# Aleph-Alpha/magma

Measured on NVIDIA H100. Metric: image-caption samples/sec (fwd+bwd), higher is better.
Workload: dtype bf16

## Files before the change

### magma_b200/csrc/attention.cu

```cuda
#include <stdlib.h>

#include "gemm_common.cuh"

namespace mb200 {

static constexpr int kAttThreads = 256;
static constexpr int kTile = 128 * 64 * 2;

struct AttnParams {
  int S, H, hd, rot;
  float scale;
  bf16* P;
  long long ldP;
  bf16* O;
  long long ldo;
  bf16* dqkv;
  long long ld_dqkv;
  const float2* rope_tab;
  const bf16* dPe;
  long long ld_dpe;
};

__device__ __forceinline__ void fence_async_smem() { asm volatile("fence.proxy.async.shared::cta;" ::: "memory"); }
__device__ __forceinline__ void wg_sync(int wg) { asm volatile("bar.sync %0, 128;" ::"r"(wg + 1) : "memory"); }

__device__ __forceinline__ uint32_t operand_off(int r, int c) {
  return (uint32_t)((c >> 6) * kTile + r * 128 + ((((c & 63) >> 3) ^ (r & 7)) << 4) + (c & 7) * 2);
}
__device__ __forceinline__ void st_pair(uint32_t saddr, float a, float b) {
  asm volatile("st.shared.b32 [%0], %1;" ::"r"(saddr), "r"(f32x2_to_bf16(a, b)) : "memory");
}
__device__ __forceinline__ float2 ld_pair(uint32_t saddr) {
  uint32_t u;
  asm volatile("ld.shared.b32 %0, [%1];" : "=r"(u) : "r"(saddr));
  return bf16x2_to_f32(u);
}
__device__ __forceinline__ float quad_max(float v) {
  v = fmaxf(v, __shfl_xor_sync(0xffffffffu, v, 1));
  return fmaxf(v, __shfl_xor_sync(0xffffffffu, v, 2));
}
__device__ __forceinline__ float quad_sum(float v) {
  v += __shfl_xor_sync(0xffffffffu, v, 1);
  return v + __shfl_xor_sync(0xffffffffu, v, 2);
}

template <int N, bool A_MN, bool B_MN>
__device__ __forceinline__ void wg_mma(float (&d)[N / 2], int wg, uint32_t a_base, uint32_t b_base, int nkb,
                                       uint32_t acc0 = 0u) {
  a_base += A_MN ? (uint32_t)(wg * kTile) : (uint32_t)(wg * 64 * 128);
  wgmma_fence();
  for (int kb = 0; kb < nkb; ++kb) {
#pragma unroll
    for (int k = 0; k < 4; ++k) {
      const uint32_t ao = A_MN ? (uint32_t)((kb * 4 + k) * 2048) : (uint32_t)(kb * kTile + k * 32);
      const uint32_t bo = B_MN ? (uint32_t)((kb * 4 + k) * 2048) : (uint32_t)(kb * kTile + k * 32);
      const uint64_t da = make_smem_desc(a_base + ao, A_MN ? (uint32_t)kTile : 0u, 1024);
      const uint64_t db = make_smem_desc(b_base + bo, B_MN ? (uint32_t)kTile : 0u, 1024);
      wgmma_bf16<N, A_MN ? 1 : 0, B_MN ? 1 : 0>(d, da, db, ((kb | k) != 0 ? 1u : 0u) | acc0);
    }
  }
  wgmma_commit();
  wgmma_wait<0>();
}

struct Frag {
  int wg, r0, c0, quad0;
  __device__ __forceinline__ Frag() {
    const int t = threadIdx.x;
    wg = t >> 7;
    r0 = wg * 64 + ((t & 127) >> 5) * 16 + ((t & 31) >> 2);
    c0 = 2 * (t & 3);
    quad0 = (t & 3) == 0;
  }
};

template <int HD>
__device__ __forceinline__ void store_rows(const Frag& f, const float (&d)[HD / 2], bf16* dst, long long ld, int nrows,
                                           const float2* tab, int rot) {
#pragma unroll
  for (int h = 0; h < 2; ++h) {
    const int r = f.r0 + 8 * h;
    if (r >= nrows) continue;
    bf16* row = dst + (long long)r * ld;
#pragma unroll
    for (int j = 0; j < HD / 8; ++j) {
      const int c = 8 * j + f.c0;
      float a0 = d[4 * j + 2 * h], a1 = d[4 * j + 2 * h + 1];
      if (tab != nullptr && c < rot) {
        const float2 cs = __ldg(tab + (long long)r * (rot >> 1) + (c >> 1));
        const float b0 = a0 * cs.x + a1 * cs.y;
        a1 = a1 * cs.x - a0 * cs.y;
        a0 = b0;
      }
      *reinterpret_cast<uint32_t*>(row + c) = f32x2_to_bf16(a0, a1);
    }
  }
}

template <int HD>
__global__ void __launch_bounds__(kAttThreads, 1)
attn_fwd_tile_kernel(const __grid_constant__ CUtensorMap tmQ, const __grid_constant__ CUtensorMap tmK,
                     const __grid_constant__ CUtensorMap tmV, const AttnParams p) {
  extern __shared__ uint8_t smem_raw[];
  uint8_t* smem = reinterpret_cast<uint8_t*>((reinterpret_cast<uintptr_t>(smem_raw) + 1023) & ~uintptr_t(1023));
  constexpr int nhb = HD / 64;
  uint8_t* sQ = smem;
  uint8_t* sK = sQ + nhb * kTile;
  uint8_t* sV = sK + nhb * kTile;
  uint8_t* sP = sV + nhb * kTile;
  uint64_t* bars = reinterpret_cast<uint64_t*>(sP + 2 * kTile);
  uint64_t* bar_qk = bars + 0;
  uint64_t* bar_v = bars + 1;

  const int t = threadIdx.x;
  const int h = blockIdx.x % p.H, b = blockIdx.x / p.H;
  const Frag f;

  pdl_trigger();
  if (t == 0) {
    tma_prefetch_desc(&tmQ);
    tma_prefetch_desc(&tmK);
    tma_prefetch_desc(&tmV);
    for (int i = 0; i < 2; ++i) mbar_init(&bars[i], 1);
    mbar_fence_init();
  }
  __syncthreads();
  pdl_wait();

  if (t == 0) {
    mbar_expect_tx(bar_qk, 2 * nhb * kTile);
    for (int kb = 0; kb < nhb; ++kb) {
      tma_load_4d(sQ + kb * kTile, &tmQ, bar_qk, kb * 64, 0, h, b);
      tma_load_4d(sK + kb * kTile, &tmK, bar_qk, kb * 64, 0, h, b);
    }
    mbar_expect_tx(bar_v, nhb * kTile);
    for (int kb = 0; kb < nhb; ++kb) tma_load_4d(sV + kb * kTile, &tmV, bar_v, kb * 64, 0, h, b);
  }
  mbar_wait(bar_qk, 0);
  float s[64];
  wg_mma<128, false, false>(s, f.wg, smem_u32(sQ), smem_u32(sK), nhb);
  const uint32_t sP_s = smem_u32(sP);
#pragma unroll
  for (int hh = 0; hh < 2; ++hh) {
    const int q = f.r0 + 8 * hh;
    const int lim = min(p.S, q + 1);
    float m = -INFINITY;
#pragma unroll
    for (int j = 0; j < 16; ++j)
#pragma unroll
      for (int e = 0; e < 2; ++e) {
        float& v = s[4 * j + 2 * hh + e];
        v *= p.scale;
        if (8 * j + f.c0 + e < lim) m = fmaxf(m, v);
      }
    m = quad_max(m);
    float sum = 0.f;
#pragma unroll
    for (int j = 0; j < 16; ++j)
#pragma unroll
      for (int e = 0; e < 2; ++e) {
        float& v = s[4 * j + 2 * hh + e];
        v = 8 * j + f.c0 + e < lim ? __expf(v - m) : 0.f;
        sum += v;
      }
    sum = quad_sum(sum);
    const float inv = q < p.S ? 1.f / sum : 0.f;
    bf16* prow = p.P + (((long long)b * p.H + h) * p.S + q) * p.ldP;
#pragma unroll
    for (int j = 0; j < 16; ++j) {
      const int c = 8 * j + f.c0;
      const float a0 = s[4 * j + 2 * hh] * inv, a1 = s[4 * j + 2 * hh + 1] * inv;
      st_pair(sP_s + operand_off(q, c), a0, a1);
      if (q < p.S && c < p.ldP) *reinterpret_cast<uint32_t*>(prow + c) = f32x2_to_bf16(a0, a1);
    }
  }
  fence_async_smem();
  wg_sync(f.wg);
  mbar_wait(bar_v, 0);
  float o[HD / 2];
  wg_mma<HD, false, true>(o, f.wg, sP_s, smem_u32(sV), 2);
  store_rows<HD>(f, o, p.O + (long long)b * p.S * p.ldo + (long long)h * HD, p.ldo, p.S, nullptr, 0);
}

template <int HD, bool EXT_DP>
__global__ void __launch_bounds__(kAttThreads, 1)
attn_bwd_tile_kernel(const __grid_constant__ CUtensorMap tmQ, const __grid_constant__ CUtensorMap tmK,
                     const __grid_constant__ CUtensorMap tmV, const __grid_constant__ CUtensorMap tmdO,
                     const __grid_constant__ CUtensorMap tmP, const AttnParams p) {
  extern __shared__ uint8_t smem_raw[];
  uint8_t* smem = reinterpret_cast<uint8_t*>((reinterpret_cast<uintptr_t>(smem_raw) + 1023) & ~uintptr_t(1023));
  constexpr int nhb = HD / 64;
  uint8_t* R1 = smem;
  uint8_t* R2 = R1 + nhb * kTile;
  uint8_t* R3 = R2 + nhb * kTile;
  uint8_t* R4 = R3 + 2 * kTile;
  uint64_t* bars = reinterpret_cast<uint64_t*>(R4 + 2 * kTile);
  uint64_t* bar_a = bars + 0;
  uint64_t* bar_p = bars + 1;
  uint64_t* bar_k = bars + 2;
  uint64_t* bar_q = bars + 3;

  const int t = threadIdx.x;
  const int h = blockIdx.x % p.H, b = blockIdx.x / p.H;
  const Frag f;

  pdl_trigger();
  if (t == 0) {
    tma_prefetch_desc(&tmQ);
    tma_prefetch_desc(&tmK);
    tma_prefetch_desc(&tmV);
    tma_prefetch_desc(&tmdO);
    tma_prefetch_desc(&tmP);
    for (int i = 0; i < 4; ++i) mbar_init(&bars[i], 1);
    mbar_fence_init();
  }
  __syncthreads();
  pdl_wait();

  if (t == 0) {
    mbar_expect_tx(bar_a, 2 * nhb * kTile);
    for (int kb = 0; kb < nhb; ++kb) {
      tma_load_4d(R1 + kb * kTile, &tmdO, bar_a, kb * 64, 0, h, b);
      tma_load_4d(R2 + kb * kTile, &tmV, bar_a, kb * 64, 0, h, b);
    }
    mbar_expect_tx(bar_p, 2 * kTile);
    for (int kb = 0; kb < 2; ++kb) tma_load_4d(R3 + kb * kTile, &tmP, bar_p, kb * 64, 0, h, b);
  }
  const uint32_t R3_s = smem_u32(R3), R4_s = smem_u32(R4);
  {
    uint32_t ext[EXT_DP ? 32 : 1];
    if (EXT_DP) {
#pragma unroll
      for (int hh = 0; hh < 2; ++hh) {
        const int q = f.r0 + 8 * hh;
        const bf16* erow = p.dPe + (((long long)b * p.H + h) * p.S + q) * p.ld_dpe;
#pragma unroll
        for (int j = 0; j < 16; ++j) {
          const int c = 8 * j + f.c0;
          uint32_t v = 0u;
          if (q < p.S && c < p.S) {
            v = __ldg(reinterpret_cast<const unsigned int*>(erow + c));
            if (c + 1 >= p.S) v &= 0xffffu;
          }
          ext[16 * hh + j] = v;
        }
      }
    }
    mbar_wait(bar_a, 0);
    float dp[64];
    wg_mma<128, false, false>(dp, f.wg, smem_u32(R1), smem_u32(R2), nhb);
    if (EXT_DP) {
#pragma unroll
      for (int hh = 0; hh < 2; ++hh)
#pragma unroll
        for (int j = 0; j < 16; ++j) {
          const float2 e = bf16x2_to_f32(ext[16 * hh + j]);
          dp[4 * j + 2 * hh] += e.x;
          dp[4 * j + 2 * hh + 1] += e.y;
        }
    }
    mbar_wait(bar_p, 0);
#pragma unroll
    for (int hh = 0; hh < 2; ++hh) {
      const int q = f.r0 + 8 * hh;
      float acc = 0.f;
#pragma unroll
      for (int j = 0; j < 16; ++j) {
        const float2 pr = ld_pair(R3_s + operand_off(q, 8 * j + f.c0));
        acc += dp[4 * j + 2 * hh] * pr.x + dp[4 * j + 2 * hh + 1] * pr.y;
      }
      acc = quad_sum(acc);
#pragma unroll
      for (int j = 0; j < 16; ++j) {
        const uint32_t off = operand_off(q, 8 * j + f.c0);
        const float2 pr = ld_pair(R3_s + off);
        st_pair(R4_s + off, pr.x * (dp[4 * j + 2 * hh] - acc) * p.scale, pr.y * (dp[4 * j + 2 * hh + 1] - acc) * p.scale);
      }
    }
  }
  const long long HDall = (long long)p.H * HD;
  bf16* gbase = p.dqkv + (long long)b * p.S * p.ld_dqkv + (long long)h * HD;
  {
    float dv[HD / 2];
    wg_mma<HD, true, true>(dv, f.wg, R3_s, smem_u32(R1), 2);
    store_rows<HD>(f, dv, gbase + 2 * HDall, p.ld_dqkv, p.S, nullptr, 0);
  }
  fence_async_smem();
  __syncthreads();
  if (t == 0) {
    mbar_expect_tx(bar_k, nhb * kTile);
    for (int kb = 0; kb < nhb; ++kb) tma_load_4d(R2 + kb * kTile, &tmK, bar_k, kb * 64, 0, h, b);
    mbar_expect_tx(bar_q, nhb * kTile);
    for (int kb = 0; kb < nhb; ++kb) tma_load_4d(R1 + kb * kTile, &tmQ, bar_q, kb * 64, 0, h, b);
  }
  {
    mbar_wait(bar_k, 0);
    float dq[HD / 2];
    wg_mma<HD, false, true>(dq, f.wg, R4_s, smem_u32(R2), 2);
    store_rows<HD>(f, dq, gbase, p.ld_dqkv, p.S, p.rope_tab, p.rot);
  }
  {
    mbar_wait(bar_q, 0);
    float dk[HD / 2];
    wg_mma<HD, true, true>(dk, f.wg, R4_s, smem_u32(R1), 2);
    store_rows<HD>(f, dk, gbase + HDall, p.ld_dqkv, p.S, p.rope_tab, p.rot);
  }
}

struct FlashParams {
  int Sq, Sk, H, hd, causal, kv_off;
  float scale;
  bf16* O;
  long long ldo;
  bf16* P;
  long long ldP;
  float2* stats;
};

template <int HD, int NBUF>
__global__ void __launch_bounds__(kAttThreads, 1)
attn_fwd_flash_kernel(const __grid_constant__ CUtensorMap tmQ, const __grid_constant__ CUtensorMap tmK,
                      const __grid_constant__ CUtensorMap tmV, const FlashParams p) {
  extern __shared__ uint8_t smem_raw[];
  uint8_t* smem = reinterpret_cast<uint8_t*>((reinterpret_cast<uintptr_t>(smem_raw) + 1023) & ~uintptr_t(1023));
  constexpr int nhb = HD / 64;
  uint8_t* sQ = smem;
  uint8_t* sK = sQ + nhb * kTile;
  uint8_t* sV = sK + NBUF * nhb * kTile;
  uint8_t* sP = sV + NBUF * nhb * kTile;
  uint64_t* bars = reinterpret_cast<uint64_t*>(sP + 2 * kTile);
  uint64_t* bar_q = bars + 0;
  uint64_t* bar_k = bars + 1;
  uint64_t* bar_v = bars + 3;

  const int t = threadIdx.x;
  const int q0 = blockIdx.x * 128, h = blockIdx.y, b = blockIdx.z;
  const Frag f;

  pdl_trigger();
  if (t == 0) {
    tma_prefetch_desc(&tmQ);
    tma_prefetch_desc(&tmK);
    tma_prefetch_desc(&tmV);
    for (int i = 0; i < 5; ++i) mbar_init(&bars[i], 1);
    mbar_fence_init();
  }
  __syncthreads();
  pdl_wait();

  int n_kv = (p.Sk + 127) >> 7;
  if (p.causal) {
    const int last_key = min(p.Sk - 1, q0 + 127 + p.kv_off);
    n_kv = last_key < 0 ? 0 : min(n_kv, (last_key >> 7) + 1);
  }
  int row_lim[2];
  bool row_ok[2];
#pragma unroll
  for (int hh = 0; hh < 2; ++hh) {
    const int qi = q0 + f.r0 + 8 * hh;
    row_lim[hh] = !p.causal ? p.Sk : min(p.Sk, qi + p.kv_off + 1);
    row_ok[hh] = qi < p.Sq;
  }

  uint32_t ph_k[2] = {0, 0}, ph_v[2] = {0, 0};
  auto load_k = [&](int j, int buf) {
    mbar_expect_tx(&bar_k[buf], nhb * kTile);
    for (int kb = 0; kb < nhb; ++kb) tma_load_4d(sK + (buf * nhb + kb) * kTile, &tmK, &bar_k[buf], kb * 64, j * 128, h, b);
  };
  auto load_v = [&](int j, int buf) {
    mbar_expect_tx(&bar_v[buf], nhb * kTile);
    for (int kb = 0; kb < nhb; ++kb) tma_load_4d(sV + (buf * nhb + kb) * kTile, &tmV, &bar_v[buf], kb * 64, j * 128, h, b);
  };

  float m[2] = {-INFINITY, -INFINITY}, l[2] = {0.f, 0.f};
  if (t == 0 && n_kv > 0) {
    mbar_expect_tx(bar_q, nhb * kTile);
    for (int kb = 0; kb < nhb; ++kb) tma_load_4d(sQ + kb * kTile, &tmQ, bar_q, kb * 64, q0, h, b);
    load_k(0, 0);
  }
  if (n_kv > 0) mbar_wait(bar_q, 0);
  float s[64];
  for (int j = 0; j < n_kv; ++j) {
    const int buf = NBUF == 2 ? (j & 1) : 0;
    if (t == 0) {
      if (NBUF == 2 && j + 1 < n_kv) load_k(j + 1, (j + 1) & 1);
      if (NBUF == 1 && j + 1 < n_kv)
        for (int kb = 0; kb < nhb; ++kb) tma_prefetch_4d(&tmK, kb * 64, (j + 1) * 128, h, b);
    }
    mbar_wait(&bar_k[buf], ph_k[buf]);
    ph_k[buf] ^= 1;
    wg_mma<128, false, false>(s, f.wg, smem_u32(sQ), smem_u32(sK + buf * nhb * kTile), nhb);
    __syncthreads();
    if (NBUF == 1 && t == 0 && j + 1 < n_kv) load_k(j + 1, 0);
    const int kbase = j * 128;
#pragma unroll
    for (int hh = 0; hh < 2; ++hh) {
      float cm = -INFINITY;
#pragma unroll
      for (int jj = 0; jj < 16; ++jj)
#pragma unroll
        for (int e = 0; e < 2; ++e)
          if (kbase + 8 * jj + f.c0 + e < row_lim[hh]) cm = fmaxf(cm, s[4 * jj + 2 * hh + e] * p.scale);
      cm = quad_max(cm);
      if (cm > m[hh]) {
        l[hh] *= __expf(m[hh] - cm);
        m[hh] = cm;
      }
      if (m[hh] != -INFINITY) {
        float ls = 0.f;
#pragma unroll
        for (int jj = 0; jj < 16; ++jj)
#pragma unroll
          for (int e = 0; e < 2; ++e)
            if (kbase + 8 * jj + f.c0 + e < row_lim[hh]) ls += __expf(s[4 * jj + 2 * hh + e] * p.scale - m[hh]);
        l[hh] += quad_sum(ls);
      }
    }
  }
  float inv[2];
#pragma unroll
  for (int hh = 0; hh < 2; ++hh) {
    inv[hh] = (row_ok[hh] && l[hh] > 0.f) ? 1.f / l[hh] : 0.f;
    if (m[hh] == -INFINITY) m[hh] = 0.f;
    if (p.stats != nullptr && row_ok[hh] && f.quad0)
      p.stats[((long long)b * p.H + h) * p.Sq + q0 + f.r0 + 8 * hh] = make_float2(m[hh], inv[hh]);
  }

  const uint32_t sP_s = smem_u32(sP);
  if (t == 0 && n_kv > 0) {
    load_k(0, 0);
    load_v(0, 0);
  }
  float o[HD / 2];
#pragma unroll
  for (int i = 0; i < HD / 2; ++i) o[i] = 0.f;
  for (int j = 0; j < n_kv; ++j) {
    const int buf = NBUF == 2 ? (j & 1) : 0;
    if (t == 0) {
      if (NBUF == 2 && j + 1 < n_kv) {
        load_k(j + 1, (j + 1) & 1);
        load_v(j + 1, (j + 1) & 1);
      }
      if (NBUF == 1 && j + 1 < n_kv)
        for (int kb = 0; kb < nhb; ++kb) {
          tma_prefetch_4d(&tmK, kb * 64, (j + 1) * 128, h, b);
          tma_prefetch_4d(&tmV, kb * 64, (j + 1) * 128, h, b);
        }
    }
    mbar_wait(&bar_k[buf], ph_k[buf]);
    ph_k[buf] ^= 1;
    wg_mma<128, false, false>(s, f.wg, smem_u32(sQ), smem_u32(sK + buf * nhb * kTile), nhb);
    __syncthreads();
    if (NBUF == 1 && t == 0 && j + 1 < n_kv) load_k(j + 1, 0);
    const int kbase = j * 128;
#pragma unroll
    for (int hh = 0; hh < 2; ++hh) {
      const int r = f.r0 + 8 * hh;
      bf16* prow = p.P ? p.P + (((long long)b * p.H + h) * p.Sq + q0 + r) * p.ldP : nullptr;
#pragma unroll
      for (int jj = 0; jj < 16; ++jj) {
        const int c = 8 * jj + f.c0;
        float a[2];
#pragma unroll
        for (int e = 0; e < 2; ++e)
          a[e] = kbase + c + e < row_lim[hh] ? __expf(s[4 * jj + 2 * hh + e] * p.scale - m[hh]) * inv[hh] : 0.f;
        st_pair(sP_s + operand_off(r, c), a[0], a[1]);
        if (prow != nullptr && row_ok[hh] && kbase + c < p.ldP)
          *reinterpret_cast<uint32_t*>(prow + kbase + c) = f32x2_to_bf16(a[0], a[1]);
      }
    }
    fence_async_smem();
    wg_sync(f.wg);
    mbar_wait(&bar_v[buf], ph_v[buf]);
    ph_v[buf] ^= 1;
    wg_mma<HD, false, true>(o, f.wg, sP_s, smem_u32(sV + buf * nhb * kTile), 2, 1u);
    __syncthreads();
    if (NBUF == 1 && t == 0 && j + 1 < n_kv) load_v(j + 1, 0);
  }
  store_rows<HD>(f, o, p.O + ((long long)b * p.Sq + q0) * p.ldo + (long long)h * HD, p.ldo, p.Sq - q0, nullptr, 0);
  if (p.P != nullptr && t < 128 && q0 + t < p.Sq) {
    bf16* prow = p.P + (((long long)b * p.H + h) * p.Sq + q0 + t) * p.ldP;
    for (int col = n_kv * 128; col < p.ldP; col += 8) *reinterpret_cast<uint4*>(prow + col) = make_uint4(0, 0, 0, 0);
  }
}

static int tile_map(CUtensorMap* m, const void* ptr, long long ld, long long bs0, long long bs1, int rows, int cols,
                    int H, int B) {
  mb200_operand op;
  op.ptr = ptr;
  op.ld = ld;
  op.bs0 = bs0;
  op.bs1 = bs1;
  op.mn_major = 0;
  op.static_data = 0;
  return make_operand_map(m, op, rows, cols, H, B, 128);
}

static constexpr int smem_max = 232448;

bool attn_tile_supported(int S, int hd) { return S >= 1 && S <= 128 && hd >= 64 && hd <= 256 && hd % 64 == 0; }

int attn_fwd_tile(const bf16* qkv, long long ld_qkv, bf16* P, long long ldP, bf16* O, long long ldo, int B, int S, int H,
                  int hd, cudaStream_t st) {
  MB_REQUIRE(attn_tile_supported(S, hd) && ldP % 8 == 0, MB200_E_SHAPE, "attn_fwd_tile: unsupported S=%d hd=%d", S, hd);
  CUtensorMap tq, tk, tv;
  const long long d = (long long)H * hd;
  int rc;
  if ((rc = tile_map(&tq, qkv, ld_qkv, hd, (long long)S * ld_qkv, S, hd, H, B))) return rc;
  if ((rc = tile_map(&tk, qkv + d, ld_qkv, hd, (long long)S * ld_qkv, S, hd, H, B))) return rc;
  if ((rc = tile_map(&tv, qkv + 2 * d, ld_qkv, hd, (long long)S * ld_qkv, S, hd, H, B))) return rc;
  AttnParams p;
  memset(&p, 0, sizeof(p));
  p.S = S;
  p.H = H;
  p.hd = hd;
  p.scale = 1.0f / sqrtf((float)hd);
  p.P = P;
  p.ldP = ldP;
  p.O = O;
  p.ldo = ldo;
  const int smem = (3 * (hd / 64) + 2) * kTile + 1024 + 128;
#define MB_FWD(HD)                                                                                                   \
  {                                                                                                                  \
    static bool set = false;                                                                                         \
    if (!set) {                                                                                                      \
      MB_CUDA(cudaFuncSetAttribute(attn_fwd_tile_kernel<HD>, cudaFuncAttributeMaxDynamicSharedMemorySize, smem_max)); \
      set = true;                                                                                                    \
    }                                                                                                                \
    MB_CUDA(launch_pdl(attn_fwd_tile_kernel<HD>, dim3(B * H), dim3(kAttThreads), (size_t)smem, st, tq, tk, tv, p));  \
  }
  switch (hd) {
    case 64: MB_FWD(64) break;
    case 128: MB_FWD(128) break;
    case 192: MB_FWD(192) break;
    default: MB_FWD(256) break;
  }
#undef MB_FWD
  count_launch();
  return 0;
}

int attn_bwd_tile(const bf16* qkv, long long ld_qkv, const bf16* dO, long long ld_do, const bf16* P, long long ldP,
                  const bf16* dPe, long long ld_dpe, bf16* dqkv, long long ld_dqkv, const float* rope_tab, int rot, int B,
                  int S, int H, int hd, cudaStream_t st) {
  MB_REQUIRE(attn_tile_supported(S, hd) && ldP % 8 == 0, MB200_E_SHAPE, "attn_bwd_tile: unsupported S=%d hd=%d", S, hd);
  MB_REQUIRE(dPe == nullptr || (ld_dpe >= S && ld_dpe % 8 == 0 && (reinterpret_cast<uintptr_t>(dPe) & 3) == 0),
             MB200_E_ALIGN, "attn_bwd_tile_dp: ld_dpe=%lld must be >= S and %%8, dP_ext 4-byte aligned", ld_dpe);
  CUtensorMap tq, tk, tv, tdo, tp;
  const long long d = (long long)H * hd;
  int rc;
  if ((rc = tile_map(&tq, qkv, ld_qkv, hd, (long long)S * ld_qkv, S, hd, H, B))) return rc;
  if ((rc = tile_map(&tk, qkv + d, ld_qkv, hd, (long long)S * ld_qkv, S, hd, H, B))) return rc;
  if ((rc = tile_map(&tv, qkv + 2 * d, ld_qkv, hd, (long long)S * ld_qkv, S, hd, H, B))) return rc;
  if ((rc = tile_map(&tdo, dO, ld_do, hd, (long long)S * ld_do, S, hd, H, B))) return rc;
  if ((rc = tile_map(&tp, P, ldP, (long long)S * ldP, (long long)H * S * ldP, S, S, H, B))) return rc;
  AttnParams p;
  memset(&p, 0, sizeof(p));
  p.S = S;
  p.H = H;
  p.hd = hd;
  p.rot = rot;
  p.scale = 1.0f / sqrtf((float)hd);
  p.P = const_cast<bf16*>(P);
  p.ldP = ldP;
  p.dqkv = dqkv;
  p.ld_dqkv = ld_dqkv;
  p.rope_tab = reinterpret_cast<const float2*>(rope_tab);
  p.dPe = dPe;
  p.ld_dpe = ld_dpe;
  const int smem = (2 * (hd / 64) + 4) * kTile + 1024 + 128;
#define MB_BWD(HD, EXT)                                                                                               \
  {                                                                                                                  \
    static bool set = false;                                                                                         \
    if (!set) {                                                                                                      \
      MB_CUDA(cudaFuncSetAttribute(attn_bwd_tile_kernel<HD, EXT>, cudaFuncAttributeMaxDynamicSharedMemorySize,       \
                                   smem_max));                                                                       \
      set = true;                                                                                                    \
    }                                                                                                                \
    MB_CUDA(launch_pdl(attn_bwd_tile_kernel<HD, EXT>, dim3(B * H), dim3(kAttThreads), (size_t)smem, st, tq, tk, tv,  \
                       tdo, tp, p));                                                                                 \
  }
  if (dPe == nullptr) {
    switch (hd) {
      case 64: MB_BWD(64, false) break;
      case 128: MB_BWD(128, false) break;
      case 192: MB_BWD(192, false) break;
      default: MB_BWD(256, false) break;
    }
  } else {
    switch (hd) {
      case 64: MB_BWD(64, true) break;
      case 128: MB_BWD(128, true) break;
      case 192: MB_BWD(192, true) break;
      default: MB_BWD(256, true) break;
    }
  }
#undef MB_BWD
  count_launch();
  return 0;
}

bool attn_flash_supported(int hd) { return hd >= 64 && hd <= 256 && hd % 64 == 0; }

int attn_fwd_flash(const bf16* q, long long ldq, long long q_bsh, long long q_bsb, const bf16* k, long long ldk,
                   long long k_bsh, long long k_bsb, const bf16* v, long long ldv, long long v_bsh, long long v_bsb,
                   bf16* O, long long ldo, bf16* P, long long ldP, float* stats, int B, int Sq, int Sk, int H, int hd,
                   int causal, cudaStream_t st) {
  MB_REQUIRE(attn_flash_supported(hd) && Sq >= 1 && Sk >= 1 && B >= 1 && H >= 1, MB200_E_SHAPE,
             "attn_fwd_flash: unsupported Sq=%d Sk=%d hd=%d", Sq, Sk, hd);
  MB_REQUIRE(!causal || Sk >= Sq, MB200_E_SHAPE, "attn_fwd_flash: causal needs Sk >= Sq (%d < %d)", Sk, Sq);
  MB_REQUIRE(P == nullptr || (ldP % 8 == 0 && ldP >= Sk), MB200_E_ALIGN, "attn_fwd_flash: ldP=%lld must be >= Sk and %%8",
             ldP);
  MB_REQUIRE(ldo % 8 == 0 && (reinterpret_cast<uintptr_t>(O) & 15) == 0, MB200_E_ALIGN, "attn_fwd_flash: O alignment");
  CUtensorMap tq, tk, tv;
  int rc;
  if ((rc = tile_map(&tq, q, ldq, q_bsh, q_bsb, Sq, hd, H, B))) return rc;
  if ((rc = tile_map(&tk, k, ldk, k_bsh, k_bsb, Sk, hd, H, B))) return rc;
  if ((rc = tile_map(&tv, v, ldv, v_bsh, v_bsb, Sk, hd, H, B))) return rc;
  FlashParams p;
  memset(&p, 0, sizeof(p));
  p.Sq = Sq;
  p.Sk = Sk;
  p.H = H;
  p.hd = hd;
  p.causal = causal;
  p.kv_off = Sk - Sq;
  p.scale = 1.0f / sqrtf((float)hd);
  p.O = O;
  p.ldo = ldo;
  p.P = P;
  p.ldP = ldP;
  p.stats = reinterpret_cast<float2*>(stats);
  const dim3 grid((Sq + 127) / 128, H, B);
#define MB_FLASH(HD, NB)                                                                                             \
  {                                                                                                                  \
    const int smem = ((1 + 2 * NB) * (HD / 64) + 2) * kTile + 1024 + 128;                                           \
    static bool set = false;                                                                                         \
    if (!set) {                                                                                                      \
      MB_CUDA(cudaFuncSetAttribute(attn_fwd_flash_kernel<HD, NB>, cudaFuncAttributeMaxDynamicSharedMemorySize,      \
                                   smem_max));                                                                       \
      set = true;                                                                                                    \
    }                                                                                                                \
    MB_CUDA(launch_pdl(attn_fwd_flash_kernel<HD, NB>, grid, dim3(kAttThreads), (size_t)smem, st, tq, tk, tv, p));    \
  }
  switch (hd) {
    case 64: MB_FLASH(64, 2) break;
    case 128: MB_FLASH(128, 2) break;
    case 192: MB_FLASH(192, 1) break;
    default: MB_FLASH(256, 1) break;
  }
#undef MB_FLASH
  count_launch();
  return 0;
}

}

extern "C" int mb200_attn_fwd_tile(const void* qkv, int64_t ld_qkv, void* P, int64_t ldP, void* O, int64_t ldo, int32_t B,
                                   int32_t S, int32_t H, int32_t hd, void* stream) {
  int rc = mb200::check_arch();
  if (rc) return rc;
  return mb200::attn_fwd_tile((const mb200::bf16*)qkv, ld_qkv, (mb200::bf16*)P, ldP, (mb200::bf16*)O, ldo, B, S, H, hd,
                              (cudaStream_t)stream);
}

extern "C" int mb200_attn_bwd_tile(const void* qkv, int64_t ld_qkv, const void* dO, int64_t ld_do, const void* P,
                                   int64_t ldP, void* dqkv, int64_t ld_dqkv, const float* rope_tab, int32_t rot,
                                   int32_t B, int32_t S, int32_t H, int32_t hd, void* stream) {
  int rc = mb200::check_arch();
  if (rc) return rc;
  return mb200::attn_bwd_tile((const mb200::bf16*)qkv, ld_qkv, (const mb200::bf16*)dO, ld_do, (const mb200::bf16*)P, ldP,
                              nullptr, 0, (mb200::bf16*)dqkv, ld_dqkv, rope_tab, rot, B, S, H, hd, (cudaStream_t)stream);
}

extern "C" int mb200_attn_bwd_tile_dp(const void* qkv, int64_t ld_qkv, const void* dO, int64_t ld_do, const void* P,
                                      int64_t ldP, const void* dP_ext, int64_t ld_dpe, void* dqkv, int64_t ld_dqkv,
                                      const float* rope_tab, int32_t rot, int32_t B, int32_t S, int32_t H, int32_t hd,
                                      void* stream) {
  int rc = mb200::check_arch();
  if (rc) return rc;
  MB_REQUIRE(dP_ext != nullptr, MB200_E_ARG, "attn_bwd_tile_dp: dP_ext is NULL");
  return mb200::attn_bwd_tile((const mb200::bf16*)qkv, ld_qkv, (const mb200::bf16*)dO, ld_do, (const mb200::bf16*)P, ldP,
                              (const mb200::bf16*)dP_ext, ld_dpe, (mb200::bf16*)dqkv, ld_dqkv, rope_tab, rot, B, S, H, hd,
                              (cudaStream_t)stream);
}

extern "C" int mb200_attn_fwd_flash(const void* q, int64_t ldq, int64_t q_bsh, int64_t q_bsb, const void* k, int64_t ldk,
                                    int64_t k_bsh, int64_t k_bsb, const void* v, int64_t ldv, int64_t v_bsh, int64_t v_bsb,
                                    void* O, int64_t ldo, void* P, int64_t ldP, float* stats, int32_t B, int32_t Sq,
                                    int32_t Sk, int32_t H, int32_t hd, int32_t causal, void* stream) {
  int rc = mb200::check_arch();
  if (rc) return rc;
  return mb200::attn_fwd_flash((const mb200::bf16*)q, ldq, q_bsh, q_bsb, (const mb200::bf16*)k, ldk, k_bsh, k_bsb,
                               (const mb200::bf16*)v, ldv, v_bsh, v_bsb, (mb200::bf16*)O, ldo, (mb200::bf16*)P, ldP, stats,
                               B, Sq, Sk, H, hd, causal, (cudaStream_t)stream);
}
```

Before: 159.7.

## Add short-sequence non-causal attention kernel with 64-row query tiles per warpgroup

Adds a specialized forward attention kernel for non-causal hd=64 with at most 384 keys. Each CTA loads all K and V for a head once, and three warpgroups each process independent 64-row query blocks with double-buffered Q loads. Softmax uses a two-pass approach (stats pass, then recompute QK for probabilities) with ex2.approx. The aim is better occupancy and K/V reuse for short cross-attention, at the cost of computing QK twice and using approximate exp.

```diff
diff --git a/magma_b200/csrc/attention.cu b/magma_b200/csrc/attention.cu
--- a/magma_b200/csrc/attention.cu
+++ b/magma_b200/csrc/attention.cu
@@ -1,4 +1,6 @@
 #include <stdlib.h>
+
+#include <type_traits>
 
 #include "gemm_common.cuh"
 
@@ -24,8 +26,8 @@
 __device__ __forceinline__ void fence_async_smem() { asm volatile("fence.proxy.async.shared::cta;" ::: "memory"); }
 __device__ __forceinline__ void wg_sync(int wg) { asm volatile("bar.sync %0, 128;" ::"r"(wg + 1) : "memory"); }
 
-__device__ __forceinline__ uint32_t operand_off(int r, int c) {
-  return (uint32_t)((c >> 6) * kTile + r * 128 + ((((c & 63) >> 3) ^ (r & 7)) << 4) + (c & 7) * 2);
+__device__ __forceinline__ uint32_t operand_off(int r, int c, int kb_bytes = kTile) {
+  return (uint32_t)((c >> 6) * kb_bytes + r * 128 + ((((c & 63) >> 3) ^ (r & 7)) << 4) + (c & 7) * 2);
 }
 __device__ __forceinline__ void st_pair(uint32_t saddr, float a, float b) {
   asm volatile("st.shared.b32 [%0], %1;" ::"r"(saddr), "r"(f32x2_to_bf16(a, b)) : "memory");
@@ -46,13 +48,13 @@
 
 template <int N, bool A_MN, bool B_MN>
 __device__ __forceinline__ void wg_mma(float (&d)[N / 2], int wg, uint32_t a_base, uint32_t b_base, int nkb,
-                                       uint32_t acc0 = 0u) {
+                                       uint32_t acc0 = 0u, uint32_t a_kb = kTile) {
   a_base += A_MN ? (uint32_t)(wg * kTile) : (uint32_t)(wg * 64 * 128);
   wgmma_fence();
   for (int kb = 0; kb < nkb; ++kb) {
 #pragma unroll
     for (int k = 0; k < 4; ++k) {
-      const uint32_t ao = A_MN ? (uint32_t)((kb * 4 + k) * 2048) : (uint32_t)(kb * kTile + k * 32);
+      const uint32_t ao = A_MN ? (uint32_t)((kb * 4 + k) * 2048) : (uint32_t)(kb * a_kb + k * 32);
       const uint32_t bo = B_MN ? (uint32_t)((kb * 4 + k) * 2048) : (uint32_t)(kb * kTile + k * 32);
       const uint64_t da = make_smem_desc(a_base + ao, A_MN ? (uint32_t)kTile : 0u, 1024);
       const uint64_t db = make_smem_desc(b_base + bo, B_MN ? (uint32_t)kTile : 0u, 1024);
@@ -484,8 +486,183 @@
   }
 }
 
+__device__ __forceinline__ float exp_ftz(float x) {
+  float y;
+  asm("ex2.approx.ftz.f32 %0, %1;" : "=f"(y) : "f"(x * 1.4426950408889634f));
+  return y;
+}
+
+static constexpr int kShortMaxKeys = 384;
+static constexpr int kShortWgs = 3;
+static constexpr int kBlk64 = 64 * 64 * 2;
+static constexpr int kShortWgBytes = 4 * kBlk64;
+
+template <int NW>
+__global__ void __launch_bounds__(NW * 128, 1)
+attn_fwd_short_kernel(const __grid_constant__ CUtensorMap tmQ, const __grid_constant__ CUtensorMap tmK,
+                      const __grid_constant__ CUtensorMap tmV, const FlashParams p, int qb_per_cta) {
+  extern __shared__ uint8_t smem_raw[];
+  uint8_t* smem = reinterpret_cast<uint8_t*>((reinterpret_cast<uintptr_t>(smem_raw) + 1023) & ~uintptr_t(1023));
+  const int n_kv = (p.Sk + 127) >> 7;
+  uint8_t* sK = smem;
+  uint8_t* sV = sK + n_kv * kTile;
+  const int t = threadIdx.x, w = t >> 7, tl = t & 127;
+  uint8_t* sQ = sV + n_kv * kTile + w * kShortWgBytes;
+  uint8_t* sP = sQ + 2 * kBlk64;
+  uint64_t* bars = reinterpret_cast<uint64_t*>(sV + n_kv * kTile + NW * kShortWgBytes);
+  uint64_t* bar_k = bars + 0;
+  uint64_t* bar_v = bars + 1;
+  uint64_t* bar_q = bars + 2 + 2 * w;
+  const int h = blockIdx.y, b = blockIdx.z;
+  const int nqb = (p.Sq + 63) >> 6;
+  const int qb0 = blockIdx.x * qb_per_cta, qb_end = min(nqb, qb0 + qb_per_cta);
+  const int rl = (tl >> 5) * 16 + ((tl & 31) >> 2);
+  const int c0 = 2 * (t & 3);
+  const bool quad0 = (t & 3) == 0;
+
+  pdl_trigger();
+  if (t == 0) {
+    tma_prefetch_desc(&tmQ);
+    tma_prefetch_desc(&tmK);
+    tma_prefetch_desc(&tmV);
+    for (int i = 0; i < 2 + 2 * NW; ++i) mbar_init(&bars[i], 1);
+    mbar_fence_init();
+  }
+  __syncthreads();
+  pdl_wait();
+
+  auto load_q = [&](int qb, int buf) {
+    mbar_expect_tx(&bar_q[buf], kBlk64);
+    tma_load_4d(sQ + buf * kBlk64, &tmQ, &bar_q[buf], 0, qb * 64, h, b);
+  };
+  if (tl == 0 && qb0 + w < qb_end) load_q(qb0 + w, 0);
+  if (t == 0) {
+    mbar_expect_tx(bar_k, n_kv * kTile);
+    for (int j = 0; j < n_kv; ++j) tma_load_4d(sK + j * kTile, &tmK, bar_k, 0, j * 128, h, b);
+    mbar_expect_tx(bar_v, n_kv * kTile);
+    for (int j = 0; j < n_kv; ++j) tma_load_4d(sV + j * kTile, &tmV, bar_v, 0, j * 128, h, b);
+  }
+  const uint32_t sK_s = smem_u32(sK), sV_s = smem_u32(sV), sP_s = smem_u32(sP);
+  float s[64];
+  int it = 0;
+  for (int qb = qb0 + w; qb < qb_end; qb += NW, ++it) {
+    const int buf = it & 1, q0 = qb * 64;
+    mbar_wait(&bar_q[buf], (it >> 1) & 1);
+    if (tl == 0 && qb + NW < qb_end) load_q(qb + NW, buf ^ 1);
+    const uint32_t sQ_s = smem_u32(sQ + buf * kBlk64);
+    bool row_ok[2];
+#pragma unroll
+    for (int hh = 0; hh < 2; ++hh) row_ok[hh] = q0 + rl + 8 * hh < p.Sq;
+    mbar_wait(bar_k, 0);
+
+    auto qk = [&](int j, int nk) {
+      if (nk > 64)
+        wg_mma<128, false, false>(s, 0, sQ_s, sK_s + j * kTile, 1);
+      else
+        wg_mma<64, false, false>(reinterpret_cast<float(&)[32]>(s), 0, sQ_s, sK_s + j * kTile, 1);
+    };
+
+    float m[2] = {-INFINITY, -INFINITY}, l[2] = {0.f, 0.f};
+    auto stats = [&](auto full, int lim) {
+      constexpr bool FULL = decltype(full)::value;
+#pragma unroll
+      for (int hh = 0; hh < 2; ++hh) {
+        float cm = -INFINITY;
+#pragma unroll
+        for (int jj = 0; jj < 16; ++jj)
+          if (FULL || 8 * jj < lim + c0)
+#pragma unroll
+            for (int e = 0; e < 2; ++e)
+              if (FULL || 8 * jj + e < lim) cm = fmaxf(cm, s[4 * jj + 2 * hh + e] * p.scale);
+        cm = quad_max(cm);
+        if (cm > m[hh]) {
+          l[hh] *= exp_ftz(m[hh] - cm);
+          m[hh] = cm;
+        }
+        if (m[hh] != -INFINITY) {
+          float ls = 0.f;
+#pragma unroll
+          for (int jj = 0; jj < 16; ++jj)
+            if (FULL || 8 * jj < lim + c0)
+#pragma unroll
+              for (int e = 0; e < 2; ++e)
+                if (FULL || 8 * jj + e < lim) ls += exp_ftz(s[4 * jj + 2 * hh + e] * p.scale - m[hh]);
+          l[hh] += quad_sum(ls);
+        }
+      }
+    };
+    for (int j = 0; j < n_kv; ++j) {
+      const int nk = p.Sk - j * 128;
+      qk(j, nk);
+      if (nk >= 128)
+        stats(std::true_type(), 0);
+      else
+        stats(std::false_type(), nk - c0);
+    }
+    float inv[2];
+#pragma unroll
+    for (int hh = 0; hh < 2; ++hh) {
+      inv[hh] = (row_ok[hh] && l[hh] > 0.f) ? 1.f / l[hh] : 0.f;
+      if (m[hh] == -INFINITY) m[hh] = 0.f;
+      if (p.stats != nullptr && row_ok[hh] && quad0)
+        p.stats[((long long)b * p.H + h) * p.Sq + q0 + rl + 8 * hh] = make_float2(m[hh], inv[hh]);
+    }
+
+    float o[32];
+#pragma unroll
+    for (int i = 0; i < 32; ++i) o[i] = 0.f;
+    bf16* prow[2];
+#pragma unroll
+    for (int hh = 0; hh < 2; ++hh)
+      prow[hh] = p.P != nullptr && row_ok[hh] ? p.P + (((long long)b * p.H + h) * p.Sq + q0 + rl + 8 * hh) * p.ldP : nullptr;
+    auto probs = [&](auto full, int kbase, int lim) {
+      constexpr bool FULL = decltype(full)::value;
+#pragma unroll
+      for (int hh = 0; hh < 2; ++hh) {
+        const int r = rl + 8 * hh;
+#pragma unroll
+        for (int jj = 0; jj < 16; ++jj) {
+          const int c = 8 * jj + c0;
+          float a[2] = {0.f, 0.f};
+          if (FULL || 8 * jj < lim + c0)
+#pragma unroll
+            for (int e = 0; e < 2; ++e)
+              if (FULL || 8 * jj + e < lim) a[e] = exp_ftz(s[4 * jj + 2 * hh + e] * p.scale - m[hh]) * inv[hh];
+          st_pair(sP_s + operand_off(r, c, kBlk64), a[0], a[1]);
+          if (prow[hh] != nullptr && (FULL || kbase + c < p.ldP))
+            *reinterpret_cast<uint32_t*>(prow[hh] + kbase + c) = f32x2_to_bf16(a[0], a[1]);
+        }
+      }
+    };
+    for (int j = 0; j < n_kv; ++j) {
+      const int kbase = j * 128, nk = p.Sk - kbase;
+      qk(j, nk);
+      wg_sync(w);
+      if (nk >= 128)
+        probs(std::true_type(), kbase, 0);
+      else
+        probs(std::false_type(), kbase, nk - c0);
+      fence_async_smem();
+      wg_sync(w);
+      mbar_wait(bar_v, 0);
+      if (nk > 64)
+        wg_mma<64, false, true>(o, 0, sP_s, sV_s + j * kTile, 2, 1u, kBlk64);
+      else
+        wg_mma<64, false, true>(o, 0, sP_s, sV_s + j * kTile, 1, 1u, kBlk64);
+    }
+    Frag f;
+    f.r0 = rl;
+    f.c0 = c0;
+    store_rows<64>(f, o, p.O + ((long long)b * p.Sq + q0) * p.ldo + (long long)h * 64, p.ldo, p.Sq - q0, nullptr, 0);
+    if (p.P != nullptr && tl < 64 && q0 + tl < p.Sq) {
+      bf16* prow = p.P + (((long long)b * p.H + h) * p.Sq + q0 + tl) * p.ldP;
+      for (int col = n_kv * 128; col < p.ldP; col += 8) *reinterpret_cast<uint4*>(prow + col) = make_uint4(0, 0, 0, 0);
+    }
+  }
+}
+
 static int tile_map(CUtensorMap* m, const void* ptr, long long ld, long long bs0, long long bs1, int rows, int cols,
-                    int H, int B) {
+                    int H, int B, int box_rows = 128) {
   mb200_operand op;
   op.ptr = ptr;
   op.ld = ld;
@@ -493,7 +670,7 @@
   op.bs1 = bs1;
   op.mn_major = 0;
   op.static_data = 0;
-  return make_operand_map(m, op, rows, cols, H, B, 128);
+  return make_operand_map(m, op, rows, cols, H, B, box_rows);
 }
 
 static constexpr int smem_max = 232448;
@@ -631,6 +808,25 @@
   p.P = P;
   p.ldP = ldP;
   p.stats = reinterpret_cast<float2*>(stats);
+  if (!causal && hd == 64 && Sk <= kShortMaxKeys) {
+    const int nqb = (Sq + 63) / 64;
+    const int qb_per_cta =
+        (long long)B * H * ((nqb + kShortWgs - 1) / kShortWgs) <= num_sms() ? kShortWgs : 2 * kShortWgs;
+    CUtensorMap tq64;
+    if ((rc = tile_map(&tq64, q, ldq, q_bsh, q_bsb, Sq, hd, H, B, 64))) return rc;
+    const int n_kv = (Sk + 127) / 128;
+    const int smem = 2 * n_kv * kTile + kShortWgs * kShortWgBytes + 1024 + 128;
+    static bool set = false;
+    if (!set) {
+      MB_CUDA(cudaFuncSetAttribute(attn_fwd_short_kernel<kShortWgs>, cudaFuncAttributeMaxDynamicSharedMemorySize,
+                                   smem_max));
+      set = true;
+    }
+    MB_CUDA(launch_pdl(attn_fwd_short_kernel<kShortWgs>, dim3((nqb + qb_per_cta - 1) / qb_per_cta, H, B),
+                       dim3(kShortWgs * 128), (size_t)smem, st, tq64, tk, tv, p, qb_per_cta));
+    count_launch();
+    return 0;
+  }
   const dim3 grid((Sq + 127) / 128, H, B);
 #define MB_FLASH(HD, NB)                                                                                             \
   {                                                                                                                  \
```

After: 162.8, median of 6. +2.0%, better.
